# YangChenApril/AMContrast3D

Hardware: AMD Instinct MI355X
Metric: train-step points/sec (fwd+bwd) on 24k-pt S3DIS clouds (higher is better)
Workload: dtype f32; 1 GPU; PointNeXt-S + AMContrast3D-AA, S3DIS-shaped 24000-pt voxelised (0.04 m) clouds, batch 8/GPU, fwd + CE/contrast loss + bwd + clip + AdamW; global_batch=8, points=24000, parallelism=dp1, launch=hipGraph replay, batches_per_joint_fps_launch=4, geometry_queue_cus=176, feature_graph_segments=1, collectives=none, update=captured in the feature graph

## Files before the change

### amcontrast3d_amd/csrc/fps.hip

```cpp
#include "common.h"

namespace amc {

#define AMC_DPP_MAX(v, CTRL) asm("s_nop 1\n\tv_max_f32_dpp %0, %0, %0 " CTRL : "+v"(v))

__device__ __forceinline__ float row_max_f32(float v)
{
    AMC_DPP_MAX(v, "quad_perm:[1,0,3,2] row_mask:0xf bank_mask:0xf");
    AMC_DPP_MAX(v, "quad_perm:[2,3,0,1] row_mask:0xf bank_mask:0xf");
    AMC_DPP_MAX(v, "row_half_mirror row_mask:0xf bank_mask:0xf");
    AMC_DPP_MAX(v, "row_mirror row_mask:0xf bank_mask:0xf");
    return v;
}

__device__ __forceinline__ float wave_max_f32(float v)
{
    v = row_max_f32(v);
    AMC_DPP_MAX(v, "row_bcast:15 row_mask:0xa bank_mask:0xf");
    AMC_DPP_MAX(v, "row_bcast:31 row_mask:0xc bank_mask:0xf");
    return __int_as_float(__builtin_amdgcn_readlane(__float_as_int(v), 63));
}

__device__ __forceinline__ void lds_barrier()
{
    asm volatile("s_waitcnt lgkmcnt(0)\n\ts_barrier" ::: "memory");
}

__device__ __forceinline__ float wave_sum_f32(float v)
{
    for (int s = 32; s >= 1; s >>= 1) v += __shfl_xor(v, s, 64);
    return v;
}

__device__ __forceinline__ float readlane_f32(float v, int lane)
{
    return __int_as_float(__builtin_amdgcn_readlane(__float_as_int(v), lane));
}

__device__ __forceinline__ float uniform_f32(float v)
{
    return __int_as_float(__builtin_amdgcn_readfirstlane(__float_as_int(v)));
}

__device__ __forceinline__ unsigned fps_key(int k, int log2rb)
{
    const unsigned tid = (unsigned)k & ((1u << log2rb) - 1u);
    const unsigned rev = log2rb ? (__brev(tid) >> (32 - log2rb)) : 0u;
    return (rev << 20) | ((unsigned)k >> log2rb);
}
__device__ __forceinline__ int fps_unkey(unsigned key, int log2rb)
{
    const unsigned rev = key >> 20, pass = key & 0xfffffu;
    const unsigned tid = log2rb ? (__brev(rev) >> (32 - log2rb)) : 0u;
    return (int)((pass << log2rb) | tid);
}

__device__ __forceinline__ unsigned morton3_4bit(unsigned x, unsigned y, unsigned z)
{
    auto spread = [](unsigned v) { return (v & 1u) | ((v & 2u) << 2) | ((v & 4u) << 4) | ((v & 8u) << 6); };
    return spread(x) | (spread(y) << 1) | (spread(z) << 2);
}

struct FpsRecord {
    float v;
    int amb;
    int spos;
    int pad;
    float x, y, z, pad2;
};

__device__ __forceinline__ void fps_morton_sort(const float *__restrict__ pts, int n, int *__restrict__ perm, int *s_cells,
                                                float (*s_red)[6], int *s_wsum)
{
    const int tid = threadIdx.x, lane = tid & 63, wave = tid >> 6;
    const int nthreads = blockDim.x, nwaves = nthreads >> 6;
    float lo[3] = {3.4e38f, 3.4e38f, 3.4e38f}, hi[3] = {-3.4e38f, -3.4e38f, -3.4e38f};
    for (int k = tid; k < n; k += nthreads) {
#pragma unroll
        for (int c = 0; c < 3; ++c) {
            const float v = pts[(size_t)k * 3 + c];
            lo[c] = fminf(lo[c], v);
            hi[c] = fmaxf(hi[c], v);
        }
    }
#pragma unroll
    for (int c = 0; c < 3; ++c) {
        lo[c] = -wave_max_f32(-lo[c]);
        hi[c] = wave_max_f32(hi[c]);
    }
    if (lane == 0) {
#pragma unroll
        for (int c = 0; c < 3; ++c) { s_red[wave][c] = lo[c]; s_red[wave][3 + c] = hi[c]; }
    }
    for (int i = tid; i < 4096; i += nthreads) s_cells[i] = 0;
    __syncthreads();
    float mn[3], sc[3];
#pragma unroll
    for (int c = 0; c < 3; ++c) {
        float l = s_red[0][c], h = s_red[0][3 + c];
        for (int w = 1; w < nwaves; ++w) { l = fminf(l, s_red[w][c]); h = fmaxf(h, s_red[w][3 + c]); }
        mn[c] = l;
        sc[c] = h > l ? 16.f / (h - l) : 0.f;
    }
    auto cell_of = [&](int k) {
        unsigned cc[3];
#pragma unroll
        for (int c = 0; c < 3; ++c) {
            const int v = (int)((pts[(size_t)k * 3 + c] - mn[c]) * sc[c]);
            cc[c] = (unsigned)min(max(v, 0), 15);
        }
        return (int)morton3_4bit(cc[0], cc[1], cc[2]);
    };
    for (int k = tid; k < n; k += nthreads) atomicAdd(&s_cells[cell_of(k)], 1);
    __syncthreads();
    const int per = 4096 / nthreads;
    int sum = 0;
    for (int i = 0; i < per; ++i) sum += s_cells[tid * per + i];
    int inc = sum;
    for (int s = 1; s < 64; s <<= 1) {
        const int o = __shfl_up(inc, s, 64);
        if (lane >= s) inc += o;
    }
    if (lane == 63) s_wsum[wave] = inc;
    __syncthreads();
    int base = 0;
    for (int w = 0; w < wave; ++w) base += s_wsum[w];
    int run = base + inc - sum;
    for (int i = 0; i < per; ++i) {
        const int c = s_cells[tid * per + i];
        s_cells[tid * per + i] = run;
        run += c;
    }
    __syncthreads();
    for (int k = tid; k < n; k += nthreads) perm[atomicAdd(&s_cells[cell_of(k)], 1)] = k;
    __syncthreads();
}

template <int PPT>
__device__ __forceinline__ void fps_slot_coords(const float (&px)[PPT], const float (&py)[PPT], const float (&pz)[PPT], int j,
                                                int wl, float &wx, float &wy, float &wz)
{
    switch (j) {
#define AMC_FPS_CASE(J)                                                                                        \
    case J:                                                                                                    \
        if (J < PPT) {                                                                                         \
            wx = readlane_f32(px[J < PPT ? J : 0], wl);                                                        \
            wy = readlane_f32(py[J < PPT ? J : 0], wl);                                                        \
            wz = readlane_f32(pz[J < PPT ? J : 0], wl);                                                        \
        }                                                                                                      \
        break;
        AMC_FPS_CASE(0) AMC_FPS_CASE(1) AMC_FPS_CASE(2) AMC_FPS_CASE(3) AMC_FPS_CASE(4) AMC_FPS_CASE(5)
        AMC_FPS_CASE(6) AMC_FPS_CASE(7) AMC_FPS_CASE(8) AMC_FPS_CASE(9) AMC_FPS_CASE(10) AMC_FPS_CASE(11)
        AMC_FPS_CASE(12) AMC_FPS_CASE(13) AMC_FPS_CASE(14) AMC_FPS_CASE(15) AMC_FPS_CASE(16) AMC_FPS_CASE(17)
        AMC_FPS_CASE(18) AMC_FPS_CASE(19) AMC_FPS_CASE(20) AMC_FPS_CASE(21) AMC_FPS_CASE(22) AMC_FPS_CASE(23)
        AMC_FPS_CASE(24) AMC_FPS_CASE(25) AMC_FPS_CASE(26) AMC_FPS_CASE(27) AMC_FPS_CASE(28) AMC_FPS_CASE(29)
        AMC_FPS_CASE(30) AMC_FPS_CASE(31) AMC_FPS_CASE(32) AMC_FPS_CASE(33) AMC_FPS_CASE(34) AMC_FPS_CASE(35)
        AMC_FPS_CASE(36) AMC_FPS_CASE(37) AMC_FPS_CASE(38) AMC_FPS_CASE(39) AMC_FPS_CASE(40) AMC_FPS_CASE(41)
        AMC_FPS_CASE(42) AMC_FPS_CASE(43) AMC_FPS_CASE(44) AMC_FPS_CASE(45) AMC_FPS_CASE(46) AMC_FPS_CASE(47)
        AMC_FPS_CASE(48) AMC_FPS_CASE(49) AMC_FPS_CASE(50) AMC_FPS_CASE(51) AMC_FPS_CASE(52) AMC_FPS_CASE(53)
        AMC_FPS_CASE(54) AMC_FPS_CASE(55) AMC_FPS_CASE(56) AMC_FPS_CASE(57) AMC_FPS_CASE(58) AMC_FPS_CASE(59)
        AMC_FPS_CASE(60) AMC_FPS_CASE(61) AMC_FPS_CASE(62) AMC_FPS_CASE(63) AMC_FPS_CASE(64) AMC_FPS_CASE(65)
        AMC_FPS_CASE(66) AMC_FPS_CASE(67) AMC_FPS_CASE(68) AMC_FPS_CASE(69) AMC_FPS_CASE(70) AMC_FPS_CASE(71)
        AMC_FPS_CASE(72) AMC_FPS_CASE(73) AMC_FPS_CASE(74) AMC_FPS_CASE(75) AMC_FPS_CASE(76) AMC_FPS_CASE(77)
        AMC_FPS_CASE(78) AMC_FPS_CASE(79) AMC_FPS_CASE(80) AMC_FPS_CASE(81) AMC_FPS_CASE(82) AMC_FPS_CASE(83)
        AMC_FPS_CASE(84) AMC_FPS_CASE(85) AMC_FPS_CASE(86) AMC_FPS_CASE(87) AMC_FPS_CASE(88) AMC_FPS_CASE(89)
        AMC_FPS_CASE(90) AMC_FPS_CASE(91) AMC_FPS_CASE(92) AMC_FPS_CASE(93) AMC_FPS_CASE(94) AMC_FPS_CASE(95)
       
#undef AMC_FPS_CASE
        default: break;
    }
}

template <int PPT, int NG, int MAXT = 512, bool LEAN = false>
__global__ __launch_bounds__(MAXT) void fps_kernel(int n, int m, int log2rb, const float *__restrict__ dataset,
                                                   float *__restrict__ temp, int *__restrict__ idxs,
                                                   int *__restrict__ perm_ws)
{
    constexpr int GS = PPT / NG;
    static_assert(GS * NG == PPT, "PPT must be a multiple of NG");
    __shared__ int s_cells[4096];
    __shared__ float s_red[16][6];
    __shared__ int s_wsum[16];
    __shared__ FpsRecord s_rec[2][16];
    __shared__ unsigned s_key[2][16];

    const int tid = threadIdx.x, lane = tid & 63, wave = tid >> 6;
    const int nthreads = blockDim.x, nwaves = nthreads >> 6;
    const float *pts = dataset + (size_t)blockIdx.x * n * 3;
    int *perm = perm_ws + (size_t)blockIdx.x * n;
    int *out = idxs + (size_t)blockIdx.x * m;

    fps_morton_sort(pts, n, perm, s_cells, s_red, s_wsum);

    auto spos_of = [&](int j, int l) { return (((j / GS) * nwaves + wave) * GS + (j % GS)) * 64 + l; };
    float px[PPT], py[PPT], pz[PPT], pt[PPT];
#pragma unroll
    for (int j = 0; j < PPT; ++j) {
        const int s = spos_of(j, lane);
        const bool ok = s < n;
        const int k = ok ? perm[s] : 0;
        px[j] = ok ? pts[(size_t)k * 3 + 0] : 0.f;
        py[j] = ok ? pts[(size_t)k * 3 + 1] : 0.f;
        pz[j] = ok ? pts[(size_t)k * 3 + 2] : 0.f;
        pt[j] = ok ? (temp ? temp[(size_t)blockIdx.x * n + k] : 1e10f) : -2.f;
    }
    float blx = 0.f, bly = 0.f, blz = 0.f, bhx = 0.f, bhy = 0.f, bhz = 0.f, pthr = -2.f;
    float gb[NG];
    int gsl[NG];
    unsigned tiebits = 0;
#pragma unroll
    for (int g = 0; g < NG; ++g) {
        float lx = 3.4e38f, ly = 3.4e38f, lz = 3.4e38f, hx = -3.4e38f, hy = -3.4e38f, hz = -3.4e38f, mx = -2.f;
#pragma unroll
        for (int jj = 0; jj < GS; ++jj) {
            const int j = g * GS + jj;
            const bool ok = pt[j] > -1.f;
            lx = fminf(lx, ok ? px[j] : 3.4e38f); hx = fmaxf(hx, ok ? px[j] : -3.4e38f);
            ly = fminf(ly, ok ? py[j] : 3.4e38f); hy = fmaxf(hy, ok ? py[j] : -3.4e38f);
            lz = fminf(lz, ok ? pz[j] : 3.4e38f); hz = fmaxf(hz, ok ? pz[j] : -3.4e38f);
            mx = fmaxf(mx, pt[j]);
        }
        lx = -wave_max_f32(-lx); ly = -wave_max_f32(-ly); lz = -wave_max_f32(-lz);
        hx = wave_max_f32(hx); hy = wave_max_f32(hy); hz = wave_max_f32(hz);
        const float thr = wave_max_f32(mx);
        if (lane == g) {
            const bool any = thr > -1.f;
            blx = any ? lx : 0.f; bly = any ? ly : 0.f; blz = any ? lz : 0.f;
            bhx = any ? hx : 0.f; bhy = any ? hy : 0.f; bhz = any ? hz : 0.f;
            pthr = thr;
        }
        gb[g] = -1.f;
        gsl[g] = g * GS;
    }

    float x1 = pts[0], y1 = pts[1], z1 = pts[2];
    if (tid == 0) out[0] = 0;
#ifdef AMC_FPS_DIAG
    unsigned long long t_acc[5] = {0, 0, 0, 0, 0}, t_prev;
#define AMC_STAMP(i)                                                                          \
    {                                                                                         \
        unsigned long long t_now;                                                             \
        asm volatile("s_memtime %0\n\ts_waitcnt lgkmcnt(0)" : "=s"(t_now)::"memory");         \
        t_acc[i] += t_now - t_prev;                                                           \
        t_prev = t_now;                                                                       \
    }
    asm volatile("s_memtime %0\n\ts_waitcnt lgkmcnt(0)" : "=s"(t_prev)::"memory");
#else
#define AMC_STAMP(i)
#endif

    for (int it = 1; it < m; ++it) {
        const int buf = it & 1;
        const float ex = fmaxf(fmaxf(blx - x1, x1 - bhx), 0.f), ey = fmaxf(fmaxf(bly - y1, y1 - bhy), 0.f),
                    ez = fmaxf(fmaxf(blz - z1, z1 - bhz), 0.f);
        const float d2box = (ex * ex + ey * ey) + ez * ez;
        const unsigned sweep = (unsigned)__ballot(lane < NG && !(d2box * 0.99999f > pthr));
#pragma unroll
        for (int g = 0; g < NG; ++g) {
            if ((sweep >> g) & 1u) {
                float b = -1.f;
                int sl = g * GS;
                bool tie = false;
#pragma unroll
                for (int jj = 0; jj < GS; ++jj) {
                    const int j = g * GS + jj;
                    const float d = dist2_ref(px[j], py[j], pz[j], x1, y1, z1);
                    const float dm = fminf(d, pt[j]);
                    pt[j] = dm;
                    if (!LEAN) {
                        const bool gtm = dm > b, eqm = dm == b;
                        tie = gtm ? false : (tie || eqm);
                        sl = gtm ? j : sl;
                    }
                    b = fmaxf(b, dm);
                    if (GS >= 4) __builtin_amdgcn_sched_barrier(0);
                }
                gb[g] = b;
                if (!LEAN) {
                    gsl[g] = sl;
                    tiebits = tie ? (tiebits | (1u << g)) : (tiebits & ~(1u << g));
                }
                const float nthr = wave_max_f32(b);
                pthr = lane == g ? nthr : pthr;
            }
        }
        AMC_STAMP(0)
        float vw, wx = 0.f, wy = 0.f, wz = 0.f;
        bool amb_w;
        int wl, jstar;
        if (LEAN) {
            float best = gb[0];
#pragma unroll
            for (int g = 1; g < NG; ++g) best = fmaxf(best, gb[g]);
            int bg = 0, eqc = 0;
#pragma unroll
            for (int g = NG - 1; g >= 0; --g) {
                const bool eq = gb[g] == best;
                bg = eq ? g : bg;
                eqc += eq ? 1 : 0;
            }
            vw = wave_max_f32(best);
            const unsigned long long cand = __ballot(best == vw);
            wl = (int)__builtin_ctzll(cand);
            const int gstar = __builtin_amdgcn_readlane(bg, wl);
            int sl = 0, cnt = 0;
            switch (gstar) {
#define AMC_FPS_GCASE(G)                                                                                       \
    case G:                                                                                                    \
        if (G < NG) {                                                                                          \
            _Pragma("unroll") for (int jj = GS - 1; jj >= 0; --jj) {                                            \
                const int j = (G < NG ? G : 0) * GS + jj;                                                       \
                const bool eq = pt[j] == vw;                                                                    \
                sl = eq ? j : sl;                                                                               \
                cnt += eq ? 1 : 0;                                                                              \
            }                                                                                                  \
        }                                                                                                      \
        break;
                AMC_FPS_GCASE(0) AMC_FPS_GCASE(1) AMC_FPS_GCASE(2) AMC_FPS_GCASE(3) AMC_FPS_GCASE(4) AMC_FPS_GCASE(5)
                AMC_FPS_GCASE(6) AMC_FPS_GCASE(7) AMC_FPS_GCASE(8) AMC_FPS_GCASE(9) AMC_FPS_GCASE(10) AMC_FPS_GCASE(11)
                AMC_FPS_GCASE(12) AMC_FPS_GCASE(13) AMC_FPS_GCASE(14) AMC_FPS_GCASE(15)
#undef AMC_FPS_GCASE
                default: break;
            }
            jstar = __builtin_amdgcn_readlane(sl, wl);
            fps_slot_coords<PPT>(px, py, pz, jstar, wl, wx, wy, wz);
            amb_w = __popcll(cand) != 1 || __builtin_amdgcn_readlane(eqc, wl) != 1 || __builtin_amdgcn_readlane(cnt, wl) != 1;
        } else {
            float best = gb[0];
            int slot = gsl[0];
            bool ltie = (tiebits & 1u) != 0;
    #pragma unroll
            for (int g = 1; g < NG; ++g) {
                const bool gtm = gb[g] > best, eqm = gb[g] == best;
                ltie = gtm ? ((tiebits >> g) & 1u) != 0 : (ltie || eqm);
                slot = gtm ? gsl[g] : slot;
                best = fmaxf(best, gb[g]);
            }
            vw = wave_max_f32(best);
            const unsigned long long cand = __ballot(best == vw);
            amb_w = __popcll(cand) != 1 || __ballot(best == vw && ltie) != 0;
            wl = (int)__builtin_ctzll(cand);
            jstar = __builtin_amdgcn_readlane(slot, wl);
            switch (jstar) {
    #define AMC_FPS_CASE(J)                                                                                        \
        case J:                                                                                                    \
            if (J < PPT) {                                                                                         \
                wx = readlane_f32(px[J < PPT ? J : 0], wl);                                                        \
                wy = readlane_f32(py[J < PPT ? J : 0], wl);                                                        \
                wz = readlane_f32(pz[J < PPT ? J : 0], wl);                                                        \
            }                                                                                                      \
            break;
                AMC_FPS_CASE(0) AMC_FPS_CASE(1) AMC_FPS_CASE(2) AMC_FPS_CASE(3) AMC_FPS_CASE(4) AMC_FPS_CASE(5)
                AMC_FPS_CASE(6) AMC_FPS_CASE(7) AMC_FPS_CASE(8) AMC_FPS_CASE(9) AMC_FPS_CASE(10) AMC_FPS_CASE(11)
                AMC_FPS_CASE(12) AMC_FPS_CASE(13) AMC_FPS_CASE(14) AMC_FPS_CASE(15) AMC_FPS_CASE(16) AMC_FPS_CASE(17)
                AMC_FPS_CASE(18) AMC_FPS_CASE(19) AMC_FPS_CASE(20) AMC_FPS_CASE(21) AMC_FPS_CASE(22) AMC_FPS_CASE(23)
                AMC_FPS_CASE(24) AMC_FPS_CASE(25) AMC_FPS_CASE(26) AMC_FPS_CASE(27) AMC_FPS_CASE(28) AMC_FPS_CASE(29)
                AMC_FPS_CASE(30) AMC_FPS_CASE(31) AMC_FPS_CASE(32) AMC_FPS_CASE(33) AMC_FPS_CASE(34) AMC_FPS_CASE(35)
                AMC_FPS_CASE(36) AMC_FPS_CASE(37) AMC_FPS_CASE(38) AMC_FPS_CASE(39) AMC_FPS_CASE(40) AMC_FPS_CASE(41)
                AMC_FPS_CASE(42) AMC_FPS_CASE(43) AMC_FPS_CASE(44) AMC_FPS_CASE(45) AMC_FPS_CASE(46) AMC_FPS_CASE(47)
                AMC_FPS_CASE(48) AMC_FPS_CASE(49) AMC_FPS_CASE(50) AMC_FPS_CASE(51) AMC_FPS_CASE(52) AMC_FPS_CASE(53)
                AMC_FPS_CASE(54) AMC_FPS_CASE(55) AMC_FPS_CASE(56) AMC_FPS_CASE(57) AMC_FPS_CASE(58) AMC_FPS_CASE(59)
                AMC_FPS_CASE(60) AMC_FPS_CASE(61) AMC_FPS_CASE(62) AMC_FPS_CASE(63) AMC_FPS_CASE(64) AMC_FPS_CASE(65)
                AMC_FPS_CASE(66) AMC_FPS_CASE(67) AMC_FPS_CASE(68) AMC_FPS_CASE(69) AMC_FPS_CASE(70) AMC_FPS_CASE(71)
                AMC_FPS_CASE(72) AMC_FPS_CASE(73) AMC_FPS_CASE(74) AMC_FPS_CASE(75) AMC_FPS_CASE(76) AMC_FPS_CASE(77)
                AMC_FPS_CASE(78) AMC_FPS_CASE(79) AMC_FPS_CASE(80) AMC_FPS_CASE(81) AMC_FPS_CASE(82) AMC_FPS_CASE(83)
                AMC_FPS_CASE(84) AMC_FPS_CASE(85) AMC_FPS_CASE(86) AMC_FPS_CASE(87) AMC_FPS_CASE(88) AMC_FPS_CASE(89)
                AMC_FPS_CASE(90) AMC_FPS_CASE(91) AMC_FPS_CASE(92) AMC_FPS_CASE(93) AMC_FPS_CASE(94) AMC_FPS_CASE(95)
           
    #undef AMC_FPS_CASE
                default: break;
            }
        }
        if (lane == 0) {
            FpsRecord r;
            r.v = vw; r.amb = amb_w ? 1 : 0; r.spos = spos_of(jstar, wl); r.pad = 0;
            r.x = wx; r.y = wy; r.z = wz; r.pad2 = 0.f;
            s_rec[buf][wave] = r;
        }
        AMC_STAMP(1)
        lds_barrier();
        AMC_STAMP(2)
        float rv = -3.f, rx = 0.f, ry = 0.f, rz = 0.f;
        int ra = 0, rs = 0;
        if (lane < nwaves) {
            const FpsRecord r = s_rec[buf][lane];
            rv = r.v; ra = r.amb; rs = r.spos; rx = r.x; ry = r.y; rz = r.z;
        }
        const float vb = readlane_f32(row_max_f32(rv), 0);
        const unsigned long long candw = __ballot(lane < nwaves && rv == vb);
        const bool amb_b = __popcll(candw) != 1 || __ballot(lane < nwaves && rv == vb && ra != 0) != 0;
        if (!amb_b) {
            const int ww = (int)__builtin_ctzll(candw);
            x1 = readlane_f32(rx, ww);
            y1 = readlane_f32(ry, ww);
            z1 = readlane_f32(rz, ww);
            if (tid == 0) out[it] = -1 - __builtin_amdgcn_readlane(rs, ww);
        } else {
            unsigned mykey = 0xffffffffu;
            int l2 = lane;
            asm volatile("" : "+v"(l2));
#pragma unroll
            for (int j = 0; j < PPT; ++j) {
                if (pt[j] == vb) {
                    const unsigned key = fps_key(perm[spos_of(j, l2)], log2rb);
                    mykey = min(mykey, key);
                }
            }
            for (int s = 32; s >= 1; s >>= 1) mykey = min(mykey, (unsigned)__shfl_xor((int)mykey, s, 64));
            if (lane == 0) s_key[buf][wave] = mykey;
            lds_barrier();
            unsigned kk = 0xffffffffu;
            for (int w = 0; w < nwaves; ++w) kk = min(kk, s_key[buf][w]);
            const int old = fps_unkey(kk, log2rb);
            x1 = uniform_f32(pts[(size_t)old * 3 + 0]);
            y1 = uniform_f32(pts[(size_t)old * 3 + 1]);
            z1 = uniform_f32(pts[(size_t)old * 3 + 2]);
            if (tid == 0) out[it] = old;
        }
        AMC_STAMP(3)
    }

    __syncthreads();
    for (int i = tid; i < m; i += nthreads) {
        const int v = out[i];
        if (v < 0) out[i] = perm[-1 - v];
    }

    if (temp) {
        int l3 = lane;
        asm volatile("" : "+v"(l3));
#pragma unroll
        for (int j = 0; j < PPT; ++j) {
            const int s = spos_of(j, l3);
            if (s < n) temp[(size_t)blockIdx.x * n + perm[s]] = pt[j];
        }
    }
#ifdef AMC_FPS_DIAG
    __syncthreads();
    if (lane == 0 && temp) {
        for (int i = 0; i < 5; ++i) temp[(size_t)blockIdx.x * n + wave * 8 + i] = (float)t_acc[i];
    }
#endif
}

constexpr int FPS_L2_GROUP = 512;
constexpr int FPS_L2_MAX = 16 * 32 * FPS_L2_GROUP;

__global__ __launch_bounds__(1024) void fps_kernel_l2(int n, int m, int log2rb, const float *__restrict__ dataset,
                                                       float *__restrict__ temp, int *__restrict__ idxs,
                                                       int *__restrict__ perm_ws, float4 *__restrict__ sorted_ws)
{
    __shared__ int s_cells[4096];
    __shared__ float s_red[16][6];
    __shared__ int s_wsum[16];
    __shared__ FpsRecord s_rec[2][16];
    __shared__ unsigned s_key[2][16];
    const int tid = threadIdx.x, lane = tid & 63, wave = tid >> 6;
    const float *pts = dataset + (size_t)blockIdx.x * n * 3;
    int *perm = perm_ws + (size_t)blockIdx.x * n;
    float4 *sp = sorted_ws + (size_t)blockIdx.x * n;
    int *out = idxs + (size_t)blockIdx.x * m;

    fps_morton_sort(pts, n, perm, s_cells, s_red, s_wsum);
    for (int s0 = tid; s0 < n; s0 += 1024) {
        const int k = perm[s0];
        sp[s0] = make_float4(pts[(size_t)k * 3], pts[(size_t)k * 3 + 1], pts[(size_t)k * 3 + 2],
                             temp ? temp[(size_t)blockIdx.x * n + k] : 1e10f);
    }
    __syncthreads();

    const int ngroups = (n + FPS_L2_GROUP - 1) / FPS_L2_GROUP;
    const int ngw = (ngroups - wave + 15) / 16;
    float blx = 0.f, bly = 0.f, blz = 0.f, bhx = 0.f, bhy = 0.f, bhz = 0.f, gm = -2.f;
    float gx = 0.f, gy = 0.f, gz = 0.f;
    int gpos = 0, gtie = 0;

    auto sweep_group = [&](int g, float x1, float y1, float z1, bool first) {
        const int base = (wave + 16 * g) * FPS_L2_GROUP;
        float4 v[8];
        float b = -1.f;
        float lx = 3.4e38f, ly = 3.4e38f, lz = 3.4e38f, hx = -3.4e38f, hy = -3.4e38f, hz = -3.4e38f;
#pragma unroll
        for (int j = 0; j < 8; ++j) {
            const int s0 = base + j * 64 + lane;
            const bool ok = s0 < n;
            v[j] = ok ? sp[s0] : make_float4(0.f, 0.f, 0.f, -2.f);
            if (!first && ok) {
                const float d = dist2_ref(v[j].x, v[j].y, v[j].z, x1, y1, z1);
                const float dm = fminf(d, v[j].w);
                if (dm != v[j].w) sp[s0].w = dm;
                v[j].w = dm;
            }
            b = fmaxf(b, v[j].w);
            if (first) {
                lx = fminf(lx, ok ? v[j].x : 3.4e38f); hx = fmaxf(hx, ok ? v[j].x : -3.4e38f);
                ly = fminf(ly, ok ? v[j].y : 3.4e38f); hy = fmaxf(hy, ok ? v[j].y : -3.4e38f);
                lz = fminf(lz, ok ? v[j].z : 3.4e38f); hz = fmaxf(hz, ok ? v[j].z : -3.4e38f);
            }
        }
        const float vw = wave_max_f32(b);
        int cnt = 0, sl = 0;
        float cx = 0.f, cy = 0.f, cz = 0.f;
#pragma unroll
        for (int j = 7; j >= 0; --j) {
            const bool eq = v[j].w == vw;
            cnt += eq ? 1 : 0;
            sl = eq ? j : sl;
            cx = eq ? v[j].x : cx; cy = eq ? v[j].y : cy; cz = eq ? v[j].z : cz;
        }
        const unsigned long long cand = __ballot(cnt > 0);
        const int wl = (int)__builtin_ctzll(cand);
        const int tie = (__popcll(cand) != 1 || __builtin_amdgcn_readlane(cnt, wl) != 1) ? 1 : 0;
        const int spos = base + __builtin_amdgcn_readlane(sl, wl) * 64 + wl;
        const float wx = readlane_f32(cx, wl), wy = readlane_f32(cy, wl), wz = readlane_f32(cz, wl);
        if (first) {
            lx = -wave_max_f32(-lx); ly = -wave_max_f32(-ly); lz = -wave_max_f32(-lz);
            hx = wave_max_f32(hx); hy = wave_max_f32(hy); hz = wave_max_f32(hz);
        }
        if (lane == g) {
            gm = vw; gtie = tie; gpos = spos; gx = wx; gy = wy; gz = wz;
            if (first) { blx = lx; bly = ly; blz = lz; bhx = hx; bhy = hy; bhz = hz; }
        }
    };
    for (int g = 0; g < ngw; ++g) sweep_group(g, 0.f, 0.f, 0.f, true);

    float x1 = pts[0], y1 = pts[1], z1 = pts[2];
    if (tid == 0) out[0] = 0;
    for (int it = 1; it < m; ++it) {
        const int buf = it & 1;
        const float ex = fmaxf(fmaxf(blx - x1, x1 - bhx), 0.f), ey = fmaxf(fmaxf(bly - y1, y1 - bhy), 0.f),
                    ez = fmaxf(fmaxf(blz - z1, z1 - bhz), 0.f);
        const float d2box = (ex * ex + ey * ey) + ez * ez;
        unsigned sweep = (unsigned)__ballot(lane < ngw && !(d2box * 0.99999f > gm));
        while (sweep) {
            const int g = (int)__builtin_ctz(sweep);
            sweep &= sweep - 1;
            sweep_group(g, x1, y1, z1, false);
        }
        const float val = lane < ngw ? gm : -3.f;
        const float vw = wave_max_f32(val);
        const unsigned long long cand = __ballot(val == vw);
        const int wl = (int)__builtin_ctzll(cand);
        const bool amb_w = __popcll(cand) != 1 || __builtin_amdgcn_readlane(gtie, wl) != 0;
        if (lane == 0) {
            FpsRecord r;
            r.v = vw; r.amb = amb_w ? 1 : 0; r.spos = __builtin_amdgcn_readlane(gpos, wl); r.pad = 0;
            r.x = readlane_f32(gx, wl); r.y = readlane_f32(gy, wl); r.z = readlane_f32(gz, wl); r.pad2 = 0.f;
            s_rec[buf][wave] = r;
        }
        lds_barrier();
        float rv = -3.f, rx = 0.f, ry = 0.f, rz = 0.f;
        int ra = 0, rs = 0;
        if (lane < 16) {
            const FpsRecord r = s_rec[buf][lane];
            rv = r.v; ra = r.amb; rs = r.spos; rx = r.x; ry = r.y; rz = r.z;
        }
        const float vb = readlane_f32(row_max_f32(rv), 0);
        const unsigned long long candw = __ballot(lane < 16 && rv == vb);
        const bool amb_b = __popcll(candw) != 1 || __ballot(lane < 16 && rv == vb && ra != 0) != 0;
        if (!amb_b) {
            const int ww = (int)__builtin_ctzll(candw);
            x1 = readlane_f32(rx, ww);
            y1 = readlane_f32(ry, ww);
            z1 = readlane_f32(rz, ww);
            if (tid == 0) out[it] = -1 - __builtin_amdgcn_readlane(rs, ww);
        } else {
            unsigned mykey = 0xffffffffu;
            for (int g = 0; g < ngw; ++g) {
                if (__builtin_amdgcn_readlane(__float_as_int(gm), g) != __float_as_int(vb)) continue;
                const int base = (wave + 16 * g) * FPS_L2_GROUP;
                for (int j = 0; j < 8; ++j) {
                    const int s0 = base + j * 64 + lane;
                    if (s0 < n && sp[s0].w == vb) mykey = min(mykey, fps_key(perm[s0], log2rb));
                }
            }
            for (int s0 = 32; s0 >= 1; s0 >>= 1) mykey = min(mykey, (unsigned)__shfl_xor((int)mykey, s0, 64));
            if (lane == 0) s_key[buf][wave] = mykey;
            lds_barrier();
            unsigned kk = 0xffffffffu;
            for (int w = 0; w < 16; ++w) kk = min(kk, s_key[buf][w]);
            const int old = fps_unkey(kk, log2rb);
            x1 = uniform_f32(pts[(size_t)old * 3 + 0]);
            y1 = uniform_f32(pts[(size_t)old * 3 + 1]);
            z1 = uniform_f32(pts[(size_t)old * 3 + 2]);
            if (tid == 0) out[it] = old;
        }
    }
    __syncthreads();
    for (int i = tid; i < m; i += 1024) {
        const int v = out[i];
        if (v < 0) out[i] = perm[-1 - v];
    }
    if (temp)
        for (int s0 = tid; s0 < n; s0 += 1024) temp[(size_t)blockIdx.x * n + perm[s0]] = sp[s0].w;
}

struct Cand {
    float v;
    int key;
    int k;
};
__device__ __forceinline__ Cand better(Cand a, Cand b)
{
    const bool take_b = (b.v > a.v) || (b.v == a.v && b.key < a.key);
    return take_b ? b : a;
}
__device__ __forceinline__ Cand shfl_xor(Cand c, int m)
{
    Cand r;
    r.v = __shfl_xor(c.v, m, 64);
    r.key = __shfl_xor(c.key, m, 64);
    r.k = __shfl_xor(c.k, m, 64);
    return r;
}

__global__ __launch_bounds__(1024) void fps_kernel_large(int n, int m, const float *__restrict__ dataset,
                                                         float *__restrict__ temp, int *__restrict__ idxs)
{
    __shared__ float s_v[16];
    __shared__ int s_key[16], s_k[16];
    const int tid = threadIdx.x, lane = tid & 63, wave = tid >> 6;
    const float *pts = dataset + (size_t)blockIdx.x * n * 3;
    float *tmp = temp + (size_t)blockIdx.x * n;
    int *out = idxs + (size_t)blockIdx.x * m;
    const int key = (int)(__brev((unsigned)tid) >> 22);
    int old = 0;
    if (tid == 0) out[0] = 0;
    for (int it = 1; it < m; ++it) {
        const float x1 = pts[(size_t)old * 3], y1 = pts[(size_t)old * 3 + 1], z1 = pts[(size_t)old * 3 + 2];
        float best = -1.f;
        int besti = 0;
        for (int k = tid; k < n; k += 1024) {
            const float d = dist2_ref(pts[(size_t)k * 3], pts[(size_t)k * 3 + 1], pts[(size_t)k * 3 + 2], x1, y1, z1);
            const float d2 = fminf(d, tmp[k]);
            tmp[k] = d2;
            besti = d2 > best ? k : besti;
            best = fmaxf(best, d2);
        }
        Cand c{best, key, besti};
#pragma unroll
        for (int s = 32; s >= 1; s >>= 1) c = better(c, shfl_xor(c, s));
        __syncthreads();
        if (lane == 0) { s_v[wave] = c.v; s_key[wave] = c.key; s_k[wave] = c.k; }
        __syncthreads();
        Cand w{-3.f, 0x7fffffff, 0};
        if (lane < 16) { w.v = s_v[lane]; w.key = s_key[lane]; w.k = s_k[lane]; }
#pragma unroll
        for (int s = 8; s >= 1; s >>= 1) w = better(w, shfl_xor(w, s));
        old = __builtin_amdgcn_readfirstlane(w.k);
        if (tid == 0) out[it] = old;
    }
}

template <int PPT, int NG, int MAXT = 512, bool LEAN = false>
static int launch_fps(int b, int n, int m, int waves, int log2rb, const float *dataset, float *temp, int *idxs,
                      int *perm, hipStream_t stream)
{
    hipLaunchKernelGGL((fps_kernel<PPT, NG, MAXT, LEAN>), dim3(b), dim3(waves * 64), 0, stream, n, m, log2rb, dataset, temp, idxs,
                       perm);
    return launch_status("amc3d_furthest_point_sampling");
}

}

using namespace amc;

AMC_API size_t amc3d_fps_workspace_bytes(int b, int n)
{
    const size_t pts = (size_t)(b > 0 ? b : 0) * (size_t)(n > 0 ? n : 0);
    return ((pts * sizeof(int) + 15) & ~(size_t)15) + (n > 24576 ? pts * sizeof(float4) : 0);
}

AMC_API int amc3d_furthest_point_sampling(int b, int n, int m, const float *dataset, float *temp, int *idxs,
                                          void *workspace, size_t workspace_bytes, void *stream_)
{
    if (b <= 0 || m <= 0) return 0;
    if (n <= 0 || !dataset || !idxs) return bad_arg("amc3d_furthest_point_sampling: bad argument");
    hipStream_t stream = (hipStream_t)stream_;
    int log2rb = 0;
    while ((2 << log2rb) <= n && log2rb < 10) ++log2rb;
    if (n > FPS_L2_MAX) {
        if (!temp) return bad_arg("amc3d_furthest_point_sampling: n > 262144 needs the temp buffer");
        hipLaunchKernelGGL(fps_kernel_large, dim3(b), dim3(1024), 0, stream, n, m, dataset, temp, idxs);
        return launch_status("amc3d_furthest_point_sampling");
    }
    if (n > 24576) {
        if (!workspace || workspace_bytes < amc3d_fps_workspace_bytes(b, n))
            return bad_arg("amc3d_furthest_point_sampling: workspace too small (amc3d_fps_workspace_bytes)");
        int *perm_l2 = (int *)workspace;
        float4 *sorted_l2 = (float4 *)((char *)workspace + (((size_t)b * n * sizeof(int) + 15) & ~(size_t)15));
        hipLaunchKernelGGL(fps_kernel_l2, dim3(b), dim3(1024), 0, stream, n, m, log2rb, dataset, temp, idxs, perm_l2,
                           sorted_l2);
        return launch_status("amc3d_furthest_point_sampling");
    }
    if (!workspace || workspace_bytes < amc3d_fps_workspace_bytes(b, n))
        return bad_arg("amc3d_furthest_point_sampling: workspace too small (amc3d_fps_workspace_bytes)");
    int *perm = (int *)workspace;
    auto waves_for = [&](int ppt) {
        int w = 1;
        while (w < 8 && w * 64 * ppt < n) w <<= 1;
        return w;
    };
    if (n > 12288) return launch_fps<48, 6, 512, true>(b, n, m, 8, log2rb, dataset, temp, idxs, perm, stream);
    if (n > 6144) return launch_fps<24, 3, 512, true>(b, n, m, 8, log2rb, dataset, temp, idxs, perm, stream);
    if (n > 3072) return launch_fps<12, 3, 512, true>(b, n, m, 8, log2rb, dataset, temp, idxs, perm, stream);
    if (n > 1536) return launch_fps<6, 3, 512, true>(b, n, m, 8, log2rb, dataset, temp, idxs, perm, stream);
    if (n > 512) return launch_fps<3, 1>(b, n, m, waves_for(3), log2rb, dataset, temp, idxs, perm, stream);
    if (n > 64) return launch_fps<2, 1>(b, n, m, waves_for(2), log2rb, dataset, temp, idxs, perm, stream);
    return launch_fps<1, 1>(b, n, m, 1, log2rb, dataset, temp, idxs, perm, stream);
}
```

### amcontrast3d_amd/pipeline.py

```python
import collections

import torch

from . import geometry


_streams = {}


def _shares_queue(a, b, cycles=3_000_000):
    import time
    torch.cuda.synchronize()
    with torch.cuda.stream(b):
        probe = torch.zeros(8, device=f"cuda:{b.device_index}")
    torch.cuda.synchronize()
    with torch.cuda.stream(a):
        torch.cuda._sleep(cycles)
    t0 = time.perf_counter()
    with torch.cuda.stream(b):
        probe.add_(1)
    b.synchronize()
    dt = time.perf_counter() - t0
    torch.cuda.synchronize()
    return dt > 0.5e-3


def _side_streams(dev):
    key = (dev.type, dev.index if dev.index is not None else torch.cuda.current_device())
    if key not in _streams:
        cur = torch.cuda.current_stream(dev)
        chosen = []
        with torch.cuda.device(dev):
            for _ in range(12):
                cand = torch.cuda.Stream(dev)
                if not any(_shares_queue(r, cand) for r in [cur] + chosen):
                    chosen.append(cand)
                if len(chosen) == 2:
                    break
            while len(chosen) < 2:
                chosen.append(torch.cuda.Stream(dev))
        _streams[key] = tuple(chosen)
    return _streams[key]


class GeometryPrefetcher:

    def __init__(self, batches, model, contrast_head, num_classes, ignore_index, ambiguity_args, depth=2):
        assert depth >= 1
        self.it = iter(batches)
        self.model, self.head = model, contrast_head
        self.num_classes, self.ignore_index, self.aargs = num_classes, ignore_index, ambiguity_args
        self.depth = depth
        self.queue = collections.deque()
        self.s_fps = self.s_rest = None
        self.exhausted = False

    def __iter__(self):
        return self

    def _launch(self, data):
        dev = data["pos"].device
        if self.s_fps is None:
            self.s_fps, self.s_rest = _side_streams(dev)
        cur = torch.cuda.current_stream(dev)
        self.s_fps.wait_stream(cur)
        with torch.cuda.stream(self.s_fps):
            fps = geometry.precompute_fps(self.model, data)
        self.s_rest.wait_stream(self.s_fps)
        with torch.cuda.stream(self.s_rest):
            plan = geometry.precompute_rest(self.model, self.head, data, fps, self.num_classes, self.ignore_index,
                                            self.aargs)
            done = torch.cuda.Event()
            done.record()
        self.queue.append((data, plan, done))

    def _fill(self):
        while not self.exhausted and len(self.queue) < self.depth + 1:
            try:
                data = next(self.it)
            except StopIteration:
                self.exhausted = True
                return
            self._launch(data)

    def __next__(self):
        self._fill()
        if not self.queue:
            raise StopIteration
        data, plan, done = self.queue.popleft()
        cur = torch.cuda.current_stream(data["pos"].device)
        cur.wait_event(done)
        geometry._walk(plan, lambda t: t.record_stream(cur) if t.is_cuda else None)
        data["_geometry"] = plan
        self._fill()
        return data


_queues = {}


def _dedicated_queues(dev, geometry_cus):
    from . import ops
    key = (dev.index if dev.index is not None else torch.cuda.current_device(), int(geometry_cus))
    if key not in _queues:
        fps = next((q[0] for k, q in _queues.items() if k[0] == key[0]), None) or ops.dedicated_stream(dev)
        _queues[key] = (fps, ops.dedicated_stream(dev, 0, geometry_cus))
    return _queues[key]


class GraphPipeline:

    def __init__(self, model, step_loss, head, optimizer, example, num_classes, ignore_index, ambiguity_args, *,
                 lanes=0, max_grad_norm=None, flat_grads=None, sync_bn=False, keep_state=True, geometry_cus=None,
                 amp_dtype=None, verbose=False, tail=None, audit=None):
        from . import ops
        self.model, self.step_loss, self.head, self.opt = model, step_loss, head, optimizer
        self.tail = tail
        import os as _os
        self.audit = bool(_os.environ.get("AMC3D_AUDIT_GRAPHS")) if audit is None else bool(audit)
        self.graph_nodes = {}
        self.ncls, self.ignore, self.aargs = num_classes, ignore_index, ambiguity_args
        self.clip, self.flatg, self.sync_bn, self.amp_dtype = max_grad_norm, flat_grads, sync_bn, amp_dtype
        self.params = [p for p in model.parameters() if p.requires_grad]
        self.dev = example["pos"].device
        self.B, self.N = example["pos"].shape[:2]
        self.keys = [k for k, v in example.items() if torch.is_tensor(v)]
        self.main = torch.cuda.current_stream(self.dev)
        assert self.main != torch.cuda.default_stream(self.dev), "GraphPipeline captures on the current stream: make a side stream current"
        self.nlevels = len(list(geometry._unwrap(model).encoder.encoder))
        snapshot = self._snapshot() if keep_state else None
        self.lanes = J = max(2, lanes if lanes > 0 else self._choose_lanes(example, verbose))
        ncu = torch.cuda.get_device_properties(self.dev).multi_processor_count
        if geometry_cus is None:
            geometry_cus = 11 * ncu // 16 if self.N <= 24576 else 0
        self.s_fps, self.s_geo = _dedicated_queues(self.dev, geometry_cus)
        self.geometry_cus = geometry_cus
        self.ev_lane = [torch.cuda.Event(), torch.cuda.Event()]
        self.ev_geo, self.ev_rot = torch.cuda.Event(), torch.cuda.Event()
        from . import schedule
        self.ev_done = [torch.cuda.Event() for _ in range(schedule.SETS)]
        self._done_recorded = [False] * schedule.SETS
        self._static_grads = None
        self._lr_dev = self._device_learning_rates()
        try:
            self._build(example)
        finally:
            self._float_learning_rates()
        if snapshot is not None:
            self._restore(snapshot)
        self.tick = 0
        self._set_valid = [False] * schedule.SETS
        self._lane_valid = [[False] * J, [False] * J]
        self._lr = tuple(g["lr"] for g in optimizer.param_groups)

    def _device_learning_rates(self):
        if type(self.opt).__name__ == "FusedAdamW" or not all(g.get("capturable", False) for g in self.opt.param_groups):
            return None
        held, self._lr_given = [], [g["lr"] for g in self.opt.param_groups]
        for g in self.opt.param_groups:
            lr = g["lr"]
            if not (torch.is_tensor(lr) and lr.device == self.dev):
                lr = torch.tensor(float(lr), dtype=torch.float32, device=self.dev)
            held.append(lr)
            g["lr"] = lr
        return held

    def _float_learning_rates(self):
        if self._lr_dev is None:
            return
        for g, t, given in zip(self.opt.param_groups, self._lr_dev, self._lr_given):
            if g["lr"] is t:
                g["lr"] = given

    def _fps_all(self, batch):
        return geometry.precompute_fps_levels(self.model, batch["pos"], 0, self.nlevels)

    def _rest(self, batch, fps):
        return geometry.precompute_rest(self.model, self.head, batch, fps, self.ncls, self.ignore, self.aargs)

    def _fwd_bwd(self, data, out):
        if self.flatg is not None:
            self.flatg.zero()
        with torch.autocast("cuda", dtype=self.amp_dtype or torch.bfloat16, enabled=self.amp_dtype is not None):
            logits, loss, parts = self.step_loss(data)
        loss.backward()
        if self.flatg is not None:
            self.flatg.gather()
        out.update(logits=logits, loss=loss, parts=parts)
        if self.tail is not None:
            with torch.no_grad():
                self.tail(out, data)

    def _update(self):
        if type(self.opt).__name__ == "FusedAdamW":
            self.opt.step(max_grad_norm=self.clip)
        else:
            if self.clip:
                torch.nn.utils.clip_grad_norm_(self.params, self.clip, norm_type=2)
            self.opt.step()

    def _copy_batch(self, dst, src):
        torch._foreach_copy_([dst[k] for k in self.keys], [src[k] for k in self.keys])

    def _ms(self, fn, reps):
        fn()
        e0, e1 = torch.cuda.Event(enable_timing=True), torch.cuda.Event(enable_timing=True)
        e0.record()
        for _ in range(reps):
            fn()
        e1.record()
        e1.synchronize()
        return e0.elapsed_time(e1) / reps

    def _choose_lanes(self, example, verbose):
        data = dict(example)
        t_fps = self._ms(lambda: geometry.precompute_fps_levels(self.model, data["pos"], 0, 2), 1)
        data["_geometry"] = geometry.precompute(self.model, self.head, data, self.ncls, self.ignore, self.aargs)
        out = {}

        def feat():
            self._fwd_bwd(data, out)
            if self.flatg is None:
                for p in self.params:
                    p.grad = None
        t_feat = self._ms(feat, 2)
        t_all = None
        if t_fps <= 1.5 * t_feat:
            lanes = 4
        else:
            t_all = self._ms(lambda: self._fps_all(data), 1)
            lanes = int(-(-t_all // max(0.28 * t_feat, 1e-3)))
            if self.N >= 100000:
                lanes = max(lanes, 24)
            lanes = int(min(24, max(3, lanes)))
        if verbose:
            import sys
            print(f"GraphPipeline: sampling chain {t_fps:.1f} ms (first level{'' if t_all is None else f', {t_all:.1f} all levels'}), "
                  f"eager feature half {t_feat:.1f} ms -> {lanes} batches per joint FPS launch", file=sys.stderr)
        return lanes

    def _snapshot(self):
        sd = {k: v.detach().clone() for k, v in self.model.state_dict().items()}
        ost = {id(t): t.detach().clone() for st in self.opt.state.values() for t in st.values() if torch.is_tensor(t)}
        return sd, ost, torch.cuda.get_rng_state(self.dev)

    def _restore(self, snapshot):
        sd, ost, rng = snapshot
        with torch.no_grad():
            for k, v in self.model.state_dict().items():
                v.copy_(sd[k])
            for st in self.opt.state.values():
                for t in st.values():
                    if torch.is_tensor(t):
                        t.copy_(ost[id(t)]) if id(t) in ost else t.zero_()
        torch.cuda.set_rng_state(rng, self.dev)

    def _build(self, example):
        from .graphs import SegmentedGraph, quiesce
        import os
        import torch.distributed as tdist
        J, B = self.lanes, self.B
        ex = {k: example[k] for k in self.keys}
        lane = lambda t, l: t[l * B:(l + 1) * B]
        self.in_J = [{k: torch.cat([v] * J) for k, v in ex.items()} for _ in range(2)]
        self.fps_J = [self._fps_all(self.in_J[j]) for j in range(2)]
        self.in_lane = [[{k: lane(v, l) for k, v in self.in_J[j].items()} for l in range(J)] for j in range(2)]
        self.fps_lane = [[geometry._walk(self.fps_J[j], lambda t, l=l: lane(t, l)) for l in range(J)] for j in range(2)]
        from . import schedule
        S = schedule.SETS
        self.set_in = [{k: v.clone() for k, v in ex.items()} for _ in range(S)]
        self.set_fps = [geometry.clone(self.fps_lane[0][0]) for _ in range(S)]
        self.out = [{} for _ in range(S)]
        data0 = dict(self.set_in[0])

        def eager_step():
            data0["_geometry"] = self._rest(self.set_in[0], self._fps_all(self.set_in[0]))
            if self.flatg is None:
                self.opt.zero_grad(set_to_none=True)
            self._fwd_bwd(data0, self.out[0])
            if self.flatg is not None:
                self.flatg.allreduce()
            self._update()
        for _ in range(3):
            eager_step()
        torch.cuda.synchronize()
        has_grad = [p.grad is not None for p in self.params]
        dist_on = tdist.is_available() and tdist.is_initialized()
        if dist_on:
            quiesce()
        if self.flatg is None:
            self.opt.zero_grad(set_to_none=True)
        mode = "thread_local" if dist_on else "global"
        self.mode = mode
        audit = self.audit

        def G():
            return torch.cuda.CUDAGraph(keep_graph=True) if audit else torch.cuda.CUDAGraph()

        def audited(g, name):
            if not audit:
                return
            counts = _graphs_mod.node_type_counts(g)
            self.graph_nodes.setdefault(name, []).append(counts)
            g.instantiate()
            if counts.get("memset") and os.environ.get("AMC3D_AUDIT_GRAPHS"):
                raise RuntimeError(f"GraphPipeline: the {name} graph holds {counts['memset']} memset node(s): {counts}")
        from . import graphs as _graphs_mod
        self.g_geo, self.rest = [G() for _ in range(S)], []
        for v in range(S):
            with torch.cuda.graph(self.g_geo[v], stream=self.s_geo, capture_error_mode=mode):
                self.rest.append(geometry.split(self._rest(self.set_in[v], self.set_fps[v]))[1])
            audited(self.g_geo[v], "geometry")
        for v, r in enumerate(self.rest):
            other = set()
            geometry._walk([[self.set_fps[u], self.set_in[u]] for u in range(S) if u != v] + [self.in_J, self.fps_J],
                           lambda t: other.add(t.untyped_storage().data_ptr()))

            def check(t):
                assert t.untyped_storage().data_ptr() not in other, "the geometry plan aliases another batch's buffers"
            geometry._walk(r, check)
        fused = type(self.opt).__name__ == "FusedAdamW"
        from . import graphs as _graphs
        self.collectives_captured = dist_on and _graphs.collectives_capturable()
        inline = self.collectives_captured or (self.flatg is None and not self.sync_bn)
        self.update_in_feature_graph = inline and (fused or all(g.get("capturable", False) for g in self.opt.param_groups))
        n_coll0 = _graphs.captured_collectives
        static = None
        if self.flatg is None:
            static = [torch.zeros_like(p) if h else None for p, h in zip(self.params, has_grad)]
            for p, g0 in zip(self.params, static):
                p.grad = g0
            self._static_grads = static
            if fused:
                self.opt.prepare()
        self.g_feat = []
        for v in range(S):
            data = dict(self.set_in[v])
            data["_geometry"] = geometry.join(self.set_fps[v], self.rest[v])

            def body(data=data, v=v):
                if static is not None:
                    for p in self.params:
                        p.grad = None
                self._fwd_bwd(data, self.out[v])
                if static is not None:
                    assert all((g0 is None) == (p.grad is None) for g0, p in zip(static, self.params)), \
                        "a parameter's gradient appeared / vanished between the warm-up and the capture"
                    pairs = [(g0, p.grad) for g0, p in zip(static, self.params) if g0 is not None]
                    torch._foreach_copy_([a for a, _ in pairs], [b for _, b in pairs])
                    for p, g0 in zip(self.params, static):
                        p.grad = g0
                if self.flatg is not None and self.collectives_captured:
                    self.flatg.allreduce()
                if self.update_in_feature_graph:
                    self._update()
            if self.sync_bn and not self.collectives_captured:
                g = SegmentedGraph(mode).capture(body, stream=self.main)
            else:
                g = G()
                kw = {"pool": self.g_feat[0].pool()} if v else {}
                with torch.cuda.graph(g, stream=self.main, capture_error_mode=mode, **kw):
                    body()
                audited(g, "features")
            self.g_feat.append(g)
            if v == 0:
                self.collectives_in_graph = _graphs.captured_collectives - n_coll0
        self.g_update = None
        if self.update_in_feature_graph:
            pass
        elif fused or all(g.get("capturable", False) for g in self.opt.param_groups):
            if fused:
                self.opt.prepare()
            self.g_update = G()
            with torch.cuda.graph(self.g_update, stream=self.main, capture_error_mode=mode):
                self._update()
            audited(self.g_update, "update")
        self.g_side = []
        for t in range(schedule.period(J)):
            plan = schedule.tick_plan(t, J)
            (jc, l), v1 = plan["consume"], plan["fill"]
            g = G()
            with torch.cuda.graph(g, stream=self.s_geo, capture_error_mode=mode):
                geometry.copy_into(self.set_fps[v1], self.fps_lane[jc][l])
                self._copy_batch(self.set_in[v1], self.in_lane[jc][l])
            audited(g, "hand_down")
            self.g_side.append(g)
        self.g_fps = [G(), G()]
        for j in range(2):
            with torch.cuda.graph(self.g_fps[j], stream=self.s_fps, capture_error_mode=mode):
                geometry.copy_into(self.fps_J[j], self._fps_all(self.in_J[j]))
            audited(self.g_fps[j], "sampling")
        torch.cuda.synchronize()

    @property
    def depth(self):
        return 2 * self.lanes

    def _critical_path(self, v0):
        captured = self.g_update is not None or self.update_in_feature_graph
        if captured:
            lr = tuple(g["lr"] for g in self.opt.param_groups)
            if lr != self._lr:
                if hasattr(self.opt, "sync_hyperparameters"):
                    self.opt.sync_hyperparameters()
                else:
                    assert self._lr_dev is not None, "a captured update whose learning rates are not in device memory"
                    for g, t in zip(self.opt.param_groups, self._lr_dev):
                        if g["lr"] is not t:
                            t.fill_(float(g["lr"]))
                self._lr = lr
        self.g_feat[v0].replay()
        if self.update_in_feature_graph:
            return
        if self.flatg is not None and not self.collectives_captured:
            self.flatg.allreduce()
        if self.g_update is not None:
            self.g_update.replay()
        else:
            self._update()

    def _tick(self, it):
        from . import schedule
        J, t = self.lanes, self.tick % schedule.period(self.lanes)
        self.tick += 1
        plan = schedule.tick_plan(t, J)
        v0, v1, (jc, l), jl = plan["train"], plan["fill"], plan["consume"], plan["launch"]
        out = None
        self.main.wait_event(self.ev_geo)
        if self._set_valid[v0]:
            self._critical_path(v0)
            out = dict(self.out[v0], target=self.set_in[v0]["y"], data=self.set_in[v0])
            self.ev_done[v0].record(self.main)
            self._done_recorded[v0] = True
        if self._done_recorded[v1]:
            self.ev_done[v1].synchronize()
        with torch.cuda.stream(self.s_geo):
            self.s_geo.wait_event(self.ev_lane[jc])
            self.g_side[t].replay()
            self._set_valid[v1], self._lane_valid[jc][l] = self._lane_valid[jc][l], False
            launch = False
            if jl is not None:
                got = 0
                if it is not None:
                    for k in range(J):
                        b = next(it, None)
                        if b is None:
                            break
                        assert b["pos"].shape[:2] == (self.B, self.N), "GraphPipeline: batches must keep the shape it was built for"
                        self._copy_batch(self.in_lane[jl][k], b)
                        got += 1
                self._lane_valid[jl] = [k < got for k in range(J)]
                launch = got > 0
            self.ev_rot.record(self.s_geo)
        if launch:
            with torch.cuda.stream(self.s_fps):
                self.s_fps.wait_event(self.ev_rot)
                self.g_fps[jl].replay()
                self.ev_lane[jl].record(self.s_fps)
        with torch.cuda.stream(self.s_geo):
            self.g_geo[v1].replay()
            self.ev_geo.record(self.s_geo)
        return out, self._set_valid[v1] or any(self._lane_valid[0]) or any(self._lane_valid[1])

    def run(self, batches):
        it = iter(batches)
        if self._static_grads is not None:
            for p, g0 in zip(self.params, self._static_grads):
                if p.grad is not g0:
                    p.grad = g0
        from . import schedule
        self.tick = 0
        self._set_valid = [False] * schedule.SETS
        self._lane_valid = [[False] * self.lanes, [False] * self.lanes]
        busy = True
        while busy:
            out, busy = self._tick(it)
            if out is not None:
                yield out

    def parts_alone(self, reps=5):
        import time

        def alone(fn, stream):
            torch.cuda.synchronize()
            t = time.perf_counter()
            with torch.cuda.stream(stream):
                for _ in range(reps):
                    fn()
            torch.cuda.synchronize()
            return round((time.perf_counter() - t) / reps * 1e3, 3)
        return {"features_ms": alone(self.g_feat[0].replay, self.main),
                "update_ms": (0.0 if self.update_in_feature_graph else
                              alone(self.g_update.replay if self.g_update is not None else self._update, self.main)),
                "fps_all_levels_joint_launch_ms": alone(self.g_fps[0].replay, self.s_fps),
                "neighbourhood_geometry_ms": alone(self.g_geo[0].replay, self.s_geo),
                "hand_down_ms": alone(self.g_side[0].replay, self.s_geo)}

    def serial_ms(self, reps=5):
        import time
        J = self.lanes
        t = 0.0
        for r in range(-1, reps):
            if r == 0:
                torch.cuda.synchronize()
                t = time.perf_counter()
            for fn, st in ((self.g_side[r % len(self.g_side)].replay, self.s_geo),
                           (self.g_fps[(r // J) % 2].replay if r % J == 0 else (lambda: None), self.s_fps),
                           (self.g_geo[r % len(self.g_geo)].replay, self.s_geo), (self.g_feat[r % len(self.g_feat)].replay, self.main)):
                with torch.cuda.stream(st):
                    fn()
                st.synchronize()
            if self.flatg is not None and not self.collectives_captured:
                self.flatg.allreduce()
            if not self.update_in_feature_graph:
                (self.g_update.replay if self.g_update is not None else self._update)()
            self.main.synchronize()
        return round((time.perf_counter() - t) / reps * 1e3, 3)

    def describe(self):
        J = self.lanes
        seg = getattr(self.g_feat[0], "segments", 1)
        return {"launch": "hipGraph replay", "batches_per_joint_fps_launch": J, "look_ahead_batches": [J + 1, 2 * J],
                "geometry_queue_cus": self.geometry_cus or "all", "feature_graph_segments": seg,
                "collectives_per_step": (self.collectives_in_graph if self.collectives_captured else
                                         getattr(self.g_feat[0], "collectives", 0) + (1 if self.flatg is not None else 0)),
                "collectives": ("recorded into the feature graph (RCCL)" if self.collectives_captured else
                                "eager, between graph segments" if (self.sync_bn or self.flatg is not None) else "none"),
                "update": ("captured in the feature graph" if self.update_in_feature_graph else
                           "captured" if self.g_update is not None else "eager"),
                "pipeline": (f"3 queues: sampling (all FPS levels of {J} future batches as one launch every {J} steps) | neighbourhood + "
                             "loss geometry of the next batch (CU-masked) | features of this batch; geometry handed over without "
                             "copies (three captured variants each; the training stream carries no event another queue waits for)")}
```

Measured before the change: 36.63 million points/s.

## Pick FPS batching lanes from measured sampling-chain vs feature-step overlap

For clouds of at most 24576 points, the number of batches per joint FPS launch is no longer taken from the old heuristic. It is now chosen by timing the FPS chain on its dedicated stream while feature graphs replay alongside, then setting lanes to margin*chain/step, clamped to 4..24. Lane buffers and the alias check move to after the feature and update graphs are captured, so the measurement can use them. This is meant to size the FPS pipeline so sampling keeps pace with the feature step. In exchange it adds startup measurement time and may use more memory for the larger joint buffers.

```diff
diff --git a/amcontrast3d_amd/csrc/fps.hip b/amcontrast3d_amd/csrc/fps.hip
--- a/amcontrast3d_amd/csrc/fps.hip
+++ b/amcontrast3d_amd/csrc/fps.hip
@@ -437,7 +437,7 @@
     }
 #ifdef AMC_FPS_DIAG
     __syncthreads();
-    if (lane == 0 && temp) {
+    if (lane == 0 && temp && wave * 8 + 5 <= n) {
         for (int i = 0; i < 5; ++i) temp[(size_t)blockIdx.x * n + wave * 8 + i] = (float)t_acc[i];
     }
 #endif
diff --git a/amcontrast3d_amd/pipeline.py b/amcontrast3d_amd/pipeline.py
--- a/amcontrast3d_amd/pipeline.py
+++ b/amcontrast3d_amd/pipeline.py
@@ -94,6 +94,41 @@
         data["_geometry"] = plan
         self._fill()
         return data
+
+
+def measure_beside(fn, stream, tick=None, ahead=2, ticks=None):
+    torch.cuda.synchronize()
+    e0, e1 = torch.cuda.Event(enable_timing=True), torch.cuda.Event(enable_timing=True)
+    marks = []
+    if tick is not None:
+        for _ in range(ahead):
+            marks.append(tick(len(marks)))
+    with torch.cuda.stream(stream):
+        e0.record(stream)
+        fn()
+        e1.record(stream)
+    while tick is not None and (not e1.query() if ticks is None else len(marks) < ticks):
+        marks.append(tick(len(marks)))
+        marks[-1 - ahead].synchronize()
+    torch.cuda.synchronize()
+    ms = e0.elapsed_time(e1)
+    at = [e0.elapsed_time(m) for m in marks]
+    inside = [t for t in at if 0.0 <= t <= ms] + [t for t in at if t > ms][:1]
+    per_tick = (inside[-1] - inside[0]) / (len(inside) - 1) if len(inside) >= 2 else None
+    return ms, per_tick
+
+
+LANES_MIN, LANES_MAX = 4, 24
+LANES_MARGIN = 1.15
+
+
+def lanes_for(chain_ms, step_ms, margin=LANES_MARGIN):
+    assert chain_ms >= 0.0 and step_ms > 0.0 and margin >= 1.0
+    need = margin * chain_ms / step_ms
+    J = LANES_MIN
+    while J < LANES_MAX and J < need:
+        J += 1
+    return J
 
 
 _queues = {}
@@ -129,7 +164,14 @@
         assert self.main != torch.cuda.default_stream(self.dev), "GraphPipeline captures on the current stream: make a side stream current"
         self.nlevels = len(list(geometry._unwrap(model).encoder.encoder))
         snapshot = self._snapshot() if keep_state else None
-        self.lanes = J = max(2, lanes if lanes > 0 else self._choose_lanes(example, verbose))
+        self.verbose = verbose
+        if lanes > 0:
+            self.lanes = max(2, lanes)
+        else:
+            self.lanes = max(2, self._choose_lanes(example, verbose and self.N > 24576))
+            if self.N <= 24576:
+                self.lanes = None
+        self.lane_timings = None
         ncu = torch.cuda.get_device_properties(self.dev).multi_processor_count
         if geometry_cus is None:
             geometry_cus = 11 * ncu // 16 if self.N <= 24576 else 0
@@ -150,7 +192,7 @@
             self._restore(snapshot)
         self.tick = 0
         self._set_valid = [False] * schedule.SETS
-        self._lane_valid = [[False] * J, [False] * J]
+        self._lane_valid = [[False] * self.lanes, [False] * self.lanes]
         self._lr = tuple(g["lr"] for g in optimizer.param_groups)
 
     def _device_learning_rates(self):
@@ -211,6 +253,35 @@
         e1.record()
         e1.synchronize()
         return e0.elapsed_time(e1) / reps
+
+    def _measure_lanes(self, dist_on):
+        import statistics
+        from . import schedule
+        S = schedule.SETS
+        snapshot = self._snapshot()
+        for v in range(S):
+            with torch.cuda.stream(self.s_geo):
+                self.g_geo[v].replay()
+        torch.cuda.synchronize()
+
+        def tick(i):
+            self._critical_path(i % S)
+            ev = torch.cuda.Event(enable_timing=True)
+            ev.record(self.main)
+            return ev
+        self._lr = tuple(g["lr"] for g in self.opt.param_groups)
+        got = [measure_beside(lambda: self._fps_all(self.set_in[0]), self.s_fps, tick, ticks=8 if dist_on else None)
+               for _ in range(4)][1:]
+        self._restore(snapshot)
+        chain_ms = statistics.median(c for c, _ in got)
+        steps = [s for _, s in got if s is not None]
+        step_ms = statistics.median(steps) if steps else chain_ms
+        self.lanes = lanes_for(chain_ms, step_ms)
+        self.lane_timings = (chain_ms, step_ms)
+        if self.verbose:
+            import sys
+            print(f"GraphPipeline: sampling chain {chain_ms:.2f} ms beside the feature graph, feature replay {step_ms:.2f} ms "
+                  f"meanwhile -> {self.lanes} batches per joint FPS launch", file=sys.stderr)
 
     def _choose_lanes(self, example, verbose):
         data = dict(example)
@@ -259,17 +330,14 @@
         from .graphs import SegmentedGraph, quiesce
         import os
         import torch.distributed as tdist
-        J, B = self.lanes, self.B
+        B = self.B
         ex = {k: example[k] for k in self.keys}
         lane = lambda t, l: t[l * B:(l + 1) * B]
-        self.in_J = [{k: torch.cat([v] * J) for k, v in ex.items()} for _ in range(2)]
-        self.fps_J = [self._fps_all(self.in_J[j]) for j in range(2)]
-        self.in_lane = [[{k: lane(v, l) for k, v in self.in_J[j].items()} for l in range(J)] for j in range(2)]
-        self.fps_lane = [[geometry._walk(self.fps_J[j], lambda t, l=l: lane(t, l)) for l in range(J)] for j in range(2)]
         from . import schedule
         S = schedule.SETS
         self.set_in = [{k: v.clone() for k, v in ex.items()} for _ in range(S)]
-        self.set_fps = [geometry.clone(self.fps_lane[0][0]) for _ in range(S)]
+        fps_ex = self._fps_all(ex)
+        self.set_fps = [geometry.clone(fps_ex) for _ in range(S)]
         self.out = [{} for _ in range(S)]
         data0 = dict(self.set_in[0])
 
@@ -311,14 +379,6 @@
             with torch.cuda.graph(self.g_geo[v], stream=self.s_geo, capture_error_mode=mode):
                 self.rest.append(geometry.split(self._rest(self.set_in[v], self.set_fps[v]))[1])
             audited(self.g_geo[v], "geometry")
-        for v, r in enumerate(self.rest):
-            other = set()
-            geometry._walk([[self.set_fps[u], self.set_in[u]] for u in range(S) if u != v] + [self.in_J, self.fps_J],
-                           lambda t: other.add(t.untyped_storage().data_ptr()))
-
-            def check(t):
-                assert t.untyped_storage().data_ptr() not in other, "the geometry plan aliases another batch's buffers"
-            geometry._walk(r, check)
         fused = type(self.opt).__name__ == "FusedAdamW"
         from . import graphs as _graphs
         self.collectives_captured = dist_on and _graphs.collectives_capturable()
@@ -375,6 +435,21 @@
             with torch.cuda.graph(self.g_update, stream=self.main, capture_error_mode=mode):
                 self._update()
             audited(self.g_update, "update")
+        if self.lanes is None:
+            self._measure_lanes(dist_on)
+        J = self.lanes
+        self.in_J = [{k: torch.cat([v] * J) for k, v in ex.items()} for _ in range(2)]
+        self.fps_J = [self._fps_all(self.in_J[j]) for j in range(2)]
+        self.in_lane = [[{k: lane(v, l) for k, v in self.in_J[j].items()} for l in range(J)] for j in range(2)]
+        self.fps_lane = [[geometry._walk(self.fps_J[j], lambda t, l=l: lane(t, l)) for l in range(J)] for j in range(2)]
+        for v, r in enumerate(self.rest):
+            other = set()
+            geometry._walk([[self.set_fps[u], self.set_in[u]] for u in range(S) if u != v] + [self.in_J, self.fps_J],
+                           lambda t: other.add(t.untyped_storage().data_ptr()))
+
+            def check(t):
+                assert t.untyped_storage().data_ptr() not in other, "the geometry plan aliases another batch's buffers"
+            geometry._walk(r, check)
         self.g_side = []
         for t in range(schedule.period(J)):
             plan = schedule.tick_plan(t, J)
```

Result: no change. 36.62 million points/s (-0.0%).
